# Lain-Iwakuro/Plonky2-Demo

Hardware: AMD Instinct MI355X
Metric: proofs/sec for m=64 matmul circuit (full prove(), PoseidonGoldilocksConfig, standard_recursion_config) (higher is better)
Workload: dtype u64 (Goldilocks, 64-bit modular integer)

## Files before the change

plonky2_demo_amd/csrc/merkle.hip:

```cpp
#include "context.hpp"
#include "poseidon.cuh"
#include "keccak.cuh"
#include "host_circuit.hpp"
#include <cstring>
#include <memory>

struct gl_merkle {
    gl_ctx* ctx = nullptr;
    GlMerkle tree;
    gl_t* leaves = nullptr;
    size_t num_leaves = 0, leaf_len = 0;
};

#define GL_COOP_MAX_NODES_DEFAULT 8192u
#define GL_COOP_MAX_NODES_THROUGHPUT 1024u
static uint32_t gl_coop_max_nodes() {
    static const long env = [] { const char* e = getenv("GL_COOP_MAX_NODES"); return e ? (long)strtoul(e, nullptr, 10) : -1L; }();
    if (env >= 0) return (uint32_t)env;
    return gl_proofs_in_flight.load(std::memory_order_relaxed) > 2 ? GL_COOP_MAX_NODES_THROUGHPUT : GL_COOP_MAX_NODES_DEFAULT;
}

__device__ __forceinline__ uint32_t d_bitrev(uint32_t x, uint32_t bits) { return bits ? (__brev(x) >> (32 - bits)) : 0; }

template <int WPE>
__global__ __launch_bounds__(256, WPE) void k_merkle_leaves(const gl_t* __restrict__ base, const uint64_t* __restrict__ offsets,
                                                       uint32_t leaf_len, uint32_t lg_leaves, gl_t* __restrict__ digests) {
    const uint32_t n = 1u << lg_leaves, gid = blockIdx.x * blockDim.x + threadIdx.x, r = gid < n ? gid : n - 1;
    gl_t s[12];
#pragma unroll
    for (int i = 0; i < 12; i++) s[i] = 0;
    if (leaf_len <= 4) {
        for (uint32_t e = 0; e < leaf_len; e++) s[e] = gl_canon(base[offsets[e] + r]);
    } else {
        for (uint32_t e0 = 0; e0 < leaf_len; e0 += 8) {
            const uint32_t c = leaf_len - e0 < 8 ? leaf_len - e0 : 8;
#pragma unroll
            for (int i = 0; i < 8; i++)
                if ((uint32_t)i < c) s[i] = base[offsets[e0 + i] + r];
            psd_permute_layer<PSD_LAYER_HASH>(s);
        }
    }
    if (gid >= n) return;
    const uint32_t j = d_bitrev(r, lg_leaves);
    ulonglong2* out = reinterpret_cast<ulonglong2*>(digests + 4ull * j);
    out[0] = make_ulonglong2(gl_canon(s[0]), gl_canon(s[1]));
    out[1] = make_ulonglong2(gl_canon(s[2]), gl_canon(s[3]));
}

__global__ __launch_bounds__(256, 5) void k_merkle_level(const gl_t* __restrict__ child, gl_t* __restrict__ parent, uint32_t count) {
    const uint32_t gid = blockIdx.x * blockDim.x + threadIdx.x, i = gid < count ? gid : count - 1;
    const ulonglong2* in = reinterpret_cast<const ulonglong2*>(child + 8ull * i);
    ulonglong2 a = in[0], b = in[1], c = in[2], d = in[3];
    gl_t s[12] = {a.x, a.y, b.x, b.y, c.x, c.y, d.x, d.y, 0, 0, 0, 0};
    psd_permute_layer<PSD_LAYER_HASH>(s);
    if (gid >= count) return;
    ulonglong2* out = reinterpret_cast<ulonglong2*>(parent + 4ull * i);
    out[0] = make_ulonglong2(gl_canon(s[0]), gl_canon(s[1]));
    out[1] = make_ulonglong2(gl_canon(s[2]), gl_canon(s[3]));
}

__global__ __launch_bounds__(256) void k_merkle_level_coop(const gl_t* __restrict__ child, gl_t* __restrict__ parent, uint32_t count) {
    const uint32_t gid = blockIdx.x * blockDim.x + threadIdx.x, node = gid >> 4;
    const int l = (int)(gid & 15);
    if (node >= count) return;
    gl_t s = l < 8 ? child[8ull * node + l] : 0;
    s = psd_coop_permute(s, l);
    if (l < 4) parent[4ull * node + l] = gl_canon(s);
}
__global__ __launch_bounds__(256) void k_merkle_leaves_coop(const gl_t* __restrict__ base, const uint64_t* __restrict__ offsets,
                                                            uint32_t leaf_len, uint32_t lg_leaves, gl_t* __restrict__ digests) {
    const uint32_t gid = blockIdx.x * blockDim.x + threadIdx.x, r = gid >> 4;
    const int l = (int)(gid & 15);
    if (r >= (1u << lg_leaves)) return;
    gl_t s = 0;
    if (leaf_len <= 4) {
        if ((uint32_t)l < leaf_len) s = gl_canon(base[offsets[l] + r]);
    } else {
        for (uint32_t e0 = 0; e0 < leaf_len; e0 += 8) {
            const uint32_t c = leaf_len - e0 < 8 ? leaf_len - e0 : 8;
            if ((uint32_t)l < c) s = base[offsets[e0 + l] + r];
            s = psd_coop_permute(s, l);
        }
    }
    if (l < 4) digests[4ull * d_bitrev(r, lg_leaves) + l] = gl_canon(s);
}

#define GL_TOP_NODES 64u
__global__ __launch_bounds__(1024) void k_merkle_top_coop(gl_t* __restrict__ digests, const uint64_t* __restrict__ lev_off, uint32_t first_level,
                                                          uint32_t num_levels, uint32_t nodes_first ) {
    const uint32_t sub = blockIdx.x, g = threadIdx.x >> 4;
    const int l = (int)(threadIdx.x & 15);
    uint32_t nodes = nodes_first;
    for (uint32_t lev = first_level; lev < num_levels; lev++, nodes >>= 1) {
        const gl_t* child = digests + 4 * lev_off[lev - 1] + 8ull * sub * nodes;
        gl_t* parent = digests + 4 * lev_off[lev] + 4ull * sub * nodes;
        if (g < nodes) {
            gl_t s = l < 8 ? child[8ull * g + l] : 0;
            s = psd_coop_permute(s, l);
            if (l < 4) parent[4ull * g + l] = gl_canon(s);
        }
        __syncthreads();
    }
}

template <int LAYER, bool CANON>
__global__ __launch_bounds__(64, 5) void k_poseidon_states(gl_t* states, size_t count) {
    const size_t gid = (size_t)blockIdx.x * blockDim.x + threadIdx.x, i = gid < count ? gid : count - 1;
    gl_t s[12];
#pragma unroll
    for (int k = 0; k < 12; k++) s[k] = states[12 * i + k];
    psd_permute_layer<LAYER>(s);
// ... 72 lines not shown
        for (uint32_t e = 0; e < len; e++) h[e] = gl_canon(row[e]);
    } else {
        kck_state s;
        kck_absorb_leaf(s, len, [&](uint32_t e) { return row[e]; });
        kck_digest25(s, h);
    }
    for (int i = 0; i < 4; i++) out[4 * r + i] = h[i];
}

static int kck_merkle_levels(gl_ctx* c, const gl_t* base, const uint64_t* d_off, uint32_t leaf_len, uint32_t lg_leaves, uint32_t cap_height, GlMerkle* out) {
    const uint32_t levels = lg_leaves - cap_height + 1, n = 1u << lg_leaves;
    c->timing_begin("merkle_leaf_hash");
    hipLaunchKernelGGL(k_kck_leaves, dim3((n + 255) / 256), dim3(256), 0, c->stream, base, d_off, leaf_len, lg_leaves, out->level_ptr(0));
    c->timing_end();
    GL_CHECK_HIP(hipGetLastError());
    c->timing_begin("merkle_levels");
    uint32_t top_first = levels;
    for (uint32_t l = 1; l < levels; l++)
        if (((1u << (lg_leaves - l)) >> cap_height) <= GL_KCK_TOP_NODES) { top_first = l; break; }
    const uint64_t* d_lev_off = nullptr;
    if (top_first < levels && levels - top_first >= 2) GL_TRY(c->get_offsets_table(out->level_off.data(), out->level_off.size(), &d_lev_off));
    else top_first = levels;
    for (uint32_t l = 1; l < top_first; l++) {
        const uint32_t cnt = 1u << (lg_leaves - l);
        hipLaunchKernelGGL(k_kck_level, dim3((cnt + 255) / 256), dim3(256), 0, c->stream, out->level_ptr(l - 1), out->level_ptr(l), cnt);
    }
    if (top_first < levels)
        hipLaunchKernelGGL(k_kck_top, dim3(1u << cap_height), dim3(64), 0, c->stream, out->digests, d_lev_off, top_first, levels, (1u << (lg_leaves - top_first)) >> cap_height);
    c->timing_end();
    GL_CHECK_HIP(hipGetLastError());
    return GL_OK;
}

int gl_merkle_build(gl_ctx* c, const gl_t* base, const uint64_t* host_offsets, uint32_t leaf_len, uint32_t lg_leaves,
                    uint32_t cap_height, GlMerkle* out, uint32_t hasher) {
    GL_REQUIRE(c && base && host_offsets && out, GL_ERR_ARG, "gl_merkle_build: null argument");
    GL_REQUIRE_HASHER(hasher, "gl_merkle_build");
    GL_REQUIRE(cap_height <= lg_leaves, GL_ERR_ARG, "cap_height should be at most log2(leaves.len())");
    GL_REQUIRE(lg_leaves <= 30 && leaf_len >= 1 && leaf_len <= 4096, GL_ERR_ARG, "gl_merkle_build: unsupported shape");
    GL_TRY(c->activate());
    out->lg_leaves = lg_leaves; out->cap_height = cap_height; out->leaf_len = leaf_len; out->hasher = hasher;
    const uint32_t levels = lg_leaves - cap_height + 1;
    out->level_off.resize(levels);
    uint64_t off = 0;
    for (uint32_t l = 0; l < levels; l++) { out->level_off[l] = off; off += uint64_t(1) << (lg_leaves - l); }
    out->total_digests = off;
    GL_TRY(c->pool_alloc(off * 4 * sizeof(gl_t), (void**)&out->digests));
    const uint64_t* d_off = nullptr;
    GL_TRY(c->get_offsets_table(host_offsets, leaf_len, &d_off));
    if (hasher == GL_HASHER_KECCAK) return kck_merkle_levels(c, base, d_off, leaf_len, lg_leaves, cap_height, out);
    const uint32_t n = 1u << lg_leaves;
    const uint32_t coop = gl_coop_max_nodes();
    c->timing_begin("merkle_leaf_hash");
    if (n <= coop) hipLaunchKernelGGL(k_merkle_leaves_coop, dim3((n * 16 + 255) / 256), dim3(256), 0, c->stream, base, d_off, leaf_len, lg_leaves, out->level_ptr(0));
    else {
        static const int wpe = [] { const char* e = getenv("GL_LEAF_WPE"); return e ? atoi(e) : 5; }();
        auto kern = wpe >= 8 ? k_merkle_leaves<8> : wpe == 7 ? k_merkle_leaves<7> : wpe == 6 ? k_merkle_leaves<6> : wpe == 4 ? k_merkle_leaves<4> : k_merkle_leaves<5>;
        hipLaunchKernelGGL(kern, dim3((n + 255) / 256), dim3(256), 0, c->stream, base, d_off, leaf_len, lg_leaves, out->level_ptr(0));
    }
    c->timing_end();
    GL_CHECK_HIP(hipGetLastError());
    c->timing_begin("merkle_levels");
    uint32_t top_first = levels;
    if (coop > 0)
        for (uint32_t l = 1; l < levels; l++)
            if (((1u << (lg_leaves - l)) >> cap_height) <= GL_TOP_NODES && ((1u << (lg_leaves - l)) >> cap_height) >= 1) { top_first = l; break; }
    const uint64_t* d_lev_off = nullptr;
    if (top_first < levels && levels - top_first >= 2) GL_TRY(c->get_offsets_table(out->level_off.data(), out->level_off.size(), &d_lev_off));
    else top_first = levels;
    for (uint32_t l = 1; l < top_first; l++) {
        const uint32_t cnt = 1u << (lg_leaves - l);
        if (cnt <= coop) hipLaunchKernelGGL(k_merkle_level_coop, dim3((cnt * 16 + 255) / 256), dim3(256), 0, c->stream, out->level_ptr(l - 1), out->level_ptr(l), cnt);
        else hipLaunchKernelGGL(k_merkle_level, dim3((cnt + 255) / 256), dim3(256), 0, c->stream, out->level_ptr(l - 1), out->level_ptr(l), cnt);
    }
    if (top_first < levels)
        hipLaunchKernelGGL(k_merkle_top_coop, dim3(1u << cap_height), dim3(1024), 0, c->stream, out->digests, d_lev_off, top_first, levels,
                           (1u << (lg_leaves - top_first)) >> cap_height);
    c->timing_end();
    GL_CHECK_HIP(hipGetLastError());
    return GL_OK;
}
void gl_merkle_release(gl_ctx* c, GlMerkle* m) {
    if (m && m->digests) { c->pool_release(m->digests); m->digests = nullptr; }
}

extern "C" int gl_poseidon_permute(gl_ctx* c, uint64_t* d_states, size_t count) try {
    GL_REQUIRE(c && d_states, GL_ERR_ARG, "null argument");
    if (!count) return GL_OK;
    GL_TRY(c->activate());
    hipLaunchKernelGGL((k_poseidon_states<PSD_LAYER_HASH, true>), dim3((unsigned)((count + 63) / 64)), dim3(64), 0, c->stream, d_states, count);
    GL_CHECK_HIP(hipGetLastError());
    return GL_OK;
} catch (...) { return gl_caught(); }
extern "C" int gl_poseidon_permute_raw(gl_ctx* c, uint64_t* d_states, size_t count, int layer) try {
    GL_REQUIRE(c && d_states && (layer == PSD_LAYER_VALU || layer == PSD_LAYER_MFMA), GL_ERR_ARG, "bad argument");
    if (!count) return GL_OK;
    GL_TRY(c->activate());
    if (layer == PSD_LAYER_MFMA)
        hipLaunchKernelGGL((k_poseidon_states<PSD_LAYER_MFMA, false>), dim3((unsigned)((count + 63) / 64)), dim3(64), 0, c->stream, d_states, count);
    else
        hipLaunchKernelGGL((k_poseidon_states<PSD_LAYER_VALU, false>), dim3((unsigned)((count + 63) / 64)), dim3(64), 0, c->stream, d_states, count);
    GL_CHECK_HIP(hipGetLastError());
    return GL_OK;
} catch (...) { return gl_caught(); }
extern "C" int gl_hash_rows_h(gl_ctx* c, uint32_t hasher, const uint64_t* d_rows, size_t count, size_t len, uint64_t* d_out) try {
    GL_REQUIRE_HASHER(hasher, "gl_hash_rows_h");
    if (hasher == GL_HASHER_POSEIDON) return gl_hash_rows(c, d_rows, count, len, d_out);
    GL_REQUIRE(c && d_rows && d_out && len >= 1 && len <= 0xFFFFFFFFu, GL_ERR_ARG, "bad argument");
    if (!count) return GL_OK;
    GL_TRY(c->activate());
    hipLaunchKernelGGL(k_kck_hash_rows, dim3((unsigned)((count + 63) / 64)), dim3(64), 0, c->stream, d_rows, count, (uint32_t)len, d_out);
    GL_CHECK_HIP(hipGetLastError());
    return GL_OK;
} catch (...) { return gl_caught(); }
extern "C" int gl_hash_rows(gl_ctx* c, const uint64_t* d_rows, size_t count, size_t len, uint64_t* d_out) try {
    GL_REQUIRE(c && d_rows && d_out && len >= 1, GL_ERR_ARG, "bad argument");
    if (!count) return GL_OK;
    GL_TRY(c->activate());
    hipLaunchKernelGGL(k_hash_rows, dim3((unsigned)((count + 63) / 64)), dim3(64), 0, c->stream, d_rows, count, (uint32_t)len, d_out);
    GL_CHECK_HIP(hipGetLastError());
    return GL_OK;
} catch (...) { return gl_caught(); }

__global__ void k_rows_to_natural_cols(const gl_t* rows, uint32_t lg_rows, uint32_t cols, gl_t* out) {
    const uint64_t idx = (uint64_t)blockIdx.x * blockDim.x + threadIdx.x;
    const uint64_t nrows = uint64_t(1) << lg_rows;
// ... 72 lines not shown
```

plonky2_demo_amd/csrc/prove.hip:

```cpp
#include "context.hpp"
#include "host_circuit.hpp"
#include "fri_instance.hpp"
#include "prover_kernels.cuh"
#include "proof.hpp"
#include <cstring>
#include <memory>

using glhost::HostChallenger;
using glhost::HostCircuit;

static constexpr size_t DS_BYTES = size_t(1) << 20, DS_WORDS = DS_BYTES / sizeof(gl_t);
static constexpr size_t DS_APOW = 0, DS_APOW_WORDS = 2 * GLQ_MAX_TERMS;
static constexpr size_t DS_ZH = DS_APOW + DS_APOW_WORDS, DS_ZH_WORDS = 8;
static constexpr size_t DS_POW = DS_ZH + DS_ZH_WORDS, DS_POW_WORDS = 1;
static constexpr size_t DS_OPEN = 4096, DS_OPEN_MAX = 4096, DS_OPEN_WORDS = 2 * DS_OPEN_MAX;
static_assert(DS_POW + DS_POW_WORDS <= DS_OPEN && DS_OPEN + DS_OPEN_WORDS <= DS_WORDS, "dev_small slices overlap or do not fit");

struct gl_circuit {
    gl_ctx* ctx = nullptr;
    gl_circuit_desc desc;
    size_t n = 0;
    gl_batch* cs_batch = nullptr;
    gl_t* d_sigmas = nullptr;
    gl_t* d_l0_coset = nullptr;
// ... 441 lines not shown
    f.nnext = f.cols.size() - f.nopen;
    return f;
}

struct gl_fri {
    gl_ctx* ctx = nullptr;
    gl_fri_params params;
    std::vector<const gl_batch*> oracles;
    size_t n = 0;
    uint32_t lgN = 0;
    unsigned round = 0;
    bool committed = false;
    std::unique_ptr<DevBuf> cur_vals;
    std::unique_ptr<DevBuf> coef;
    size_t cur_n = 0; uint32_t cur_lgN = 0; gl_t shift = GL_MULT_GENERATOR;
    std::vector<std::unique_ptr<MerkleHolder>> trees;
    std::vector<std::unique_ptr<DevBuf>> vals;
    std::vector<uint32_t> lg;
    std::vector<const gl_t*> h_cols; std::vector<gl_t> h_apow;
    std::vector<const gl_t*> h_listed_cols; std::vector<gl_t> h_listed_apow;
};
extern "C" void gl_fri_free(gl_fri* f) noexcept {
    if (!f) return;
    gl_ctx* ctx = f->ctx;
    if (ctx) (void)gl_stream_wait(ctx->stream);
    delete f;
    gl_ctx_release(ctx);
}
static gl_fri_params fri_params_of(const gl_circuit_desc& d) {
    gl_fri_params p;
    p.degree_bits = d.degree_bits; p.rate_bits = d.rate_bits; p.cap_height = d.cap_height; p.proof_of_work_bits = d.proof_of_work_bits;
    p.num_query_rounds = d.num_query_rounds; p.num_fri_rounds = d.num_fri_rounds;
    for (int r = 0; r < 8; r++) p.fri_arity_bits[r] = d.fri_arity_bits[r];
    p.hiding = d.zero_knowledge; p.hasher = d.hasher;
    return p;
}
static int fri_combine(gl_ctx* ctx, const gl_circuit* cir, const gl_batch* const batches[4], const uint64_t zeta_in[2], const uint64_t alpha_in[2], gl_fri** out) {
    GL_TRY(check_phase_args(ctx, cir));
    GL_REQUIRE(batches && zeta_in && alpha_in && out, GL_ERR_ARG, "gl_fri_combine: null argument");
    const gl_circuit_desc& d = cir->desc;
    const size_t n = cir->n, N = n << d.rate_bits;
    const size_t want[4] = {d.num_constants + 80, 135, 20 + 2 * (size_t)d.num_lookup_polys, 16};
    for (int o = 0; o < 4; o++) GL_TRY(check_batch(cir, batches[o], want[o], "gl_fri_combine: oracle order is constants||sigmas, wires, Z||partial products(||lookups), quotient"));
    FriOpenings op = fri_openings(batches);
    const size_t nopen = op.nopen, nnext = op.nnext;
    hipStream_t st = ctx->stream;
    std::unique_ptr<gl_fri, void (*)(gl_fri*)> f(new gl_fri(), gl_fri_free);
    f->ctx = ctx; ctx->retain(); f->params = fri_params_of(d); f->n = n; f->lgN = d.degree_bits + d.rate_bits;
    f->oracles.assign(batches, batches + 4);
    const gl2_t zeta = gl2_make(gl_canon(zeta_in[0]), gl_canon(zeta_in[1])), fri_alpha = gl2_make(gl_canon(alpha_in[0]), gl_canon(alpha_in[1]));
    const gl2_t gzeta = gl2_canon(gl2_scalar(zeta, gl_host_root_of_unity(d.degree_bits)));
    f->coef.reset(new DevBuf(ctx)); GL_TRY(f->coef->alloc(2 * n * sizeof(gl_t)));
    {
        DevBuf d_F(ctx), d_heads(ctx), d_cols(ctx), d_apow(ctx);
        const uint32_t seg_len = (uint32_t)(n / 1024 > 32 ? n / 1024 : (n >= 32 ? 32 : n));
        const uint32_t nseg = (uint32_t)((n + seg_len - 1) / seg_len);
        GL_TRY(d_F.alloc(2 * n * sizeof(gl_t)));
        GL_TRY(d_heads.alloc(2 * (size_t)nseg * sizeof(gl_t)));
        GL_TRY(d_cols.alloc((nopen + nnext) * sizeof(gl_t*)));
        GL_TRY(d_apow.alloc(2 * (nopen + nnext) * sizeof(gl_t)));
        std::vector<const gl_t*>& cols = f->h_cols;
        cols = std::move(op.cols);
        std::vector<gl_t>& apow = f->h_apow; apow.assign(2 * (nopen + nnext), 0);
        { gl2_t x = gl2_make(1, 0); for (size_t j = 0; j < nopen; j++) { apow[2 * j] = x.a; apow[2 * j + 1] = x.b; x = gl2_canon(gl2_mul(x, fri_alpha)); } }
        gl2_t shift = gl2_make(1, 0);
        { gl2_t x = gl2_make(1, 0); for (size_t j = 0; j < nnext; j++) { apow[2 * (nopen + j)] = x.a; apow[2 * (nopen + j) + 1] = x.b; x = gl2_canon(gl2_mul(x, fri_alpha)); } shift = x; }
        GL_TRY(h2d_async(ctx, d_cols.p, cols.data(), cols.size() * sizeof(gl_t*)));
        GL_TRY(h2d_async(ctx, d_apow.p, apow.data(), apow.size() * sizeof(gl_t)));
        gl_t* Fa = d_F.as<gl_t>(); gl_t* Fb = Fa + n;
        gl_t* Qa = f->coef->as<gl_t>(); gl_t* Qb = Qa + n;
        const unsigned gb = (unsigned)((n + 63) / 64), sb = (nseg + 63) / 64;
        ctx->timing_begin("reduce batch + divide by linear");
        hipLaunchKernelGGL(k_fri_combine, dim3(gb), dim3(256), 0, st, d_cols.as<const gl_t*>(), d_apow.as<gl_t>(), (uint32_t)nopen, (uint32_t)n, Fa, Fb);
        hipLaunchKernelGGL(k_div_linear_heads, dim3(sb), dim3(64), 0, st, Fa, Fb, (uint32_t)n, seg_len, zeta.a, zeta.b, d_heads.as<gl_t>());
        hipLaunchKernelGGL(k_div_linear_carries, dim3(1), dim3(1024), 0, st, d_heads.as<gl_t>(), (uint32_t)n, seg_len, zeta.a, zeta.b);
        hipLaunchKernelGGL(k_div_linear_apply, dim3(sb), dim3(64), 0, st, Fa, Fb, (uint32_t)n, seg_len, zeta.a, zeta.b, d_heads.as<gl_t>(), shift.a, shift.b, Qa, Qb, 0);
        hipLaunchKernelGGL(k_fri_combine, dim3(gb), dim3(256), 0, st, d_cols.as<const gl_t*>() + nopen, d_apow.as<gl_t>() + 2 * nopen, (uint32_t)nnext, (uint32_t)n, Fa, Fb);
        hipLaunchKernelGGL(k_div_linear_heads, dim3(sb), dim3(64), 0, st, Fa, Fb, (uint32_t)n, seg_len, gzeta.a, gzeta.b, d_heads.as<gl_t>());
        hipLaunchKernelGGL(k_div_linear_carries, dim3(1), dim3(1024), 0, st, d_heads.as<gl_t>(), (uint32_t)n, seg_len, gzeta.a, gzeta.b);
        hipLaunchKernelGGL(k_div_linear_apply, dim3(sb), dim3(64), 0, st, Fa, Fb, (uint32_t)n, seg_len, gzeta.a, gzeta.b, d_heads.as<gl_t>(), (gl_t)1, (gl_t)0, Qa, Qb, 1);
        ctx->timing_end();
        GL_CHECK_HIP(hipGetLastError());
    }
    f->cur_vals.reset(new DevBuf(ctx)); GL_TRY(f->cur_vals->alloc(2 * N * sizeof(gl_t)));
    GL_TRY(gl_ntt_run(ctx, f->coef->as<gl_t>(), n, (uint32_t)n, f->cur_vals->as<gl_t>(), N, f->lgN, 2, false, GL_MULT_GENERATOR, 0, 1));
    f->cur_n = n; f->cur_lgN = f->lgN;
    *out = f.release();
    return GL_OK;
}
extern "C" int gl_fri_combine(gl_ctx* ctx, const gl_circuit* cir, const gl_batch* const batches[4], const uint64_t zeta_in[2], const uint64_t alpha_in[2], gl_fri** out) try {
    GL_TRY(check_phase_api(ctx, cir));
    return fri_combine(ctx, cir, batches, zeta_in, alpha_in, out);
} catch (...) { return gl_caught(); }
extern "C" int gl_fri_commit_round(gl_fri* f, uint64_t* h_cap_out) try {
    GL_REQUIRE(f && h_cap_out, GL_ERR_ARG, "gl_fri_commit_round: null argument");
    GL_REQUIRE(f->round < f->params.num_fri_rounds && !f->committed, GL_ERR_ARG, "gl_fri_commit_round: no round left to commit (call gl_fri_fold first)");
    gl_ctx* ctx = f->ctx;
    GL_TRY(ctx->activate());
    const uint32_t ab = f->params.fri_arity_bits[f->round], arity = 1u << ab;
    const size_t curN = size_t(1) << f->cur_lgN;
    std::vector<uint64_t> offs(2 * arity);
    for (uint32_t k = 0; k < arity; k++)
        for (uint32_t cpt = 0; cpt < 2; cpt++) offs[2 * k + cpt] = (uint64_t)cpt * curN + (uint64_t)host_bitrev32(k, ab) * (curN >> ab);
    std::unique_ptr<MerkleHolder> tree(new MerkleHolder(ctx));
    GL_TRY(gl_merkle_build(ctx, f->cur_vals->as<gl_t>(), offs.data(), 2 * arity, f->cur_lgN - ab, f->params.cap_height, &tree->m, f->params.hasher));
    GL_TRY(d2h(ctx, h_cap_out, tree->m.level_ptr(tree->m.num_levels() - 1), (size_t(4) << f->params.cap_height) * sizeof(gl_t)));
    f->trees.push_back(std::move(tree));
    f->committed = true;
    return GL_OK;
} catch (...) { return gl_caught(); }
extern "C" int gl_fri_fold(gl_fri* f, const uint64_t beta_in[2]) try {
    GL_REQUIRE(f && beta_in, GL_ERR_ARG, "gl_fri_fold: null argument");
    GL_REQUIRE(f->committed, GL_ERR_ARG, "gl_fri_fold: commit the round first");
    gl_ctx* ctx = f->ctx;
    GL_TRY(ctx->activate());
    const uint32_t ab = f->params.fri_arity_bits[f->round], arity = 1u << ab;
    const gl2_t beta = gl2_make(gl_canon(beta_in[0]), gl_canon(beta_in[1]));
    const size_t next_n = f->cur_n >> ab;
    GL_REQUIRE(next_n >= 1, GL_ERR_INTERNAL, "FRI fold below one coefficient");
    std::unique_ptr<DevBuf> next(new DevBuf(ctx));
    GL_TRY(next->alloc(2 * next_n * sizeof(gl_t)));
    ctx->timing_begin("fold codewords in the commitment phase");
    hipLaunchKernelGGL(k_fri_fold, dim3((unsigned)((next_n + 255) / 256)), dim3(256), 0, ctx->stream, f->coef->as<gl_t>(), f->coef->as<gl_t>() + f->cur_n,
                       (uint32_t)next_n, arity, beta.a, beta.b, next->as<gl_t>(), next->as<gl_t>() + next_n);
    ctx->timing_end();
    GL_CHECK_HIP(hipGetLastError());
    const gl_t next_shift = gl_canon(gl_exp(f->shift, arity));
    const uint32_t next_lgN = f->cur_lgN - ab;
    std::unique_ptr<DevBuf> next_vals(new DevBuf(ctx));
    GL_TRY(next_vals->alloc(2 * (size_t(1) << next_lgN) * sizeof(gl_t)));
    GL_TRY(gl_ntt_run(ctx, next->as<gl_t>(), next_n, (uint32_t)next_n, next_vals->as<gl_t>(), size_t(1) << next_lgN, next_lgN, 2, false, next_shift, 0, 1));
    f->vals.reserve(f->vals.size() + 1); f->lg.reserve(f->lg.size() + 1);
    f->vals.push_back(std::move(f->cur_vals)); f->lg.push_back(f->cur_lgN);
// ... 25 lines not shown
    GL_REQUIRE(ctx && sponge_state && witness && (input_buffer || !input_len), GL_ERR_ARG, "gl_pow_grind: null argument");
    GL_REQUIRE(input_len < 8 && min_leading_zeros <= 40, GL_ERR_ARG, "gl_pow_grind: the witness must fit the rate (input_len < 8), at most 40 bits of work");
    GL_TRY(ctx->activate());
    hipStream_t st = ctx->stream;
    GL_TRY(ctx->ensure_dev_small(DS_BYTES));
    unsigned long long* d_res = (unsigned long long*)(ctx->dev_small + DS_POW);
    GlPowParams pw;
    for (int i = 0; i < 12; i++) pw.state[i] = hasher == GL_HASHER_KECCAK ? gl_canon(sponge_state[i]) : sponge_state[i];
    for (uint32_t i = 0; i < input_len; i++) pw.state[i] = hasher == GL_HASHER_KECCAK ? gl_canon(input_buffer[i]) : input_buffer[i];
    pw.pos = input_len; pw.min_leading_zeros = min_leading_zeros; pw.result = d_res;
    static const int pow_window_env = [] { const char* e = getenv("GL_POW_WINDOW_LOG"); return e ? atoi(e) : 99; }();
    const int wlog = pow_window_env != 99 ? pow_window_env : (gl_proofs_in_flight.load(std::memory_order_relaxed) > 2 ? 0 : 1);
    const int wbits = (int)min_leading_zeros + wlog < 8 ? 8 : (int)min_leading_zeros + wlog;
    const uint64_t batch = wbits >= 30 ? (uint64_t(1) << 30) : (uint64_t(1) << wbits);
    unsigned long long res = ~0ull;
    ctx->timing_begin("find proof-of-work witness");
    for (uint64_t base = 0; base < GL_P; base += batch) {
        GL_CHECK_HIP(hipMemsetAsync(d_res, 0xFF, sizeof(unsigned long long), st));
        pw.base = base; pw.count = (GL_P - base < batch) ? GL_P - base : batch;
        if (hasher == GL_HASHER_KECCAK) hipLaunchKernelGGL(k_kck_pow_grind, dim3((unsigned)((pw.count + 255) / 256)), dim3(256), 0, st, pw);
        else hipLaunchKernelGGL(k_pow_grind, dim3((unsigned)((pw.count + 255) / 256)), dim3(256), 0, st, pw);
        GL_CHECK_HIP(hipGetLastError());
        GL_TRY(d2h(ctx, &res, d_res, sizeof res));
        if (res != ~0ull) break;
    }
    ctx->timing_end();
    GL_REQUIRE(res != ~0ull, GL_ERR_INTERNAL, "Proof of work failed. This is highly unlikely!");
    *witness = (uint64_t)res;
    return GL_OK;
} catch (...) { return gl_caught(); }

static int fri_query_blob(gl_fri* f, const uint32_t* x_index, uint32_t nq, std::vector<uint8_t>& o) {
    gl_ctx* ctx = f->ctx;
    const gl_fri_params& d = f->params;
    const size_t no = f->oracles.size();
    hipStream_t st = ctx->stream;
    const uint32_t lgN = f->lgN;
    const size_t N = size_t(1) << lgN;
    GL_REQUIRE(f->round == d.num_fri_rounds && !f->committed, GL_ERR_ARG, "gl_fri_query: reduction rounds not finished");
    for (uint32_t q = 0; q < nq; q++) GL_REQUIRE(x_index[q] < N, GL_ERR_ARG, "gl_fri_query: query index out of range");
    struct Piece { size_t off, words; };
    std::vector<Piece> row_piece(no), path_piece(no), fleaf_piece(d.num_fri_rounds), fpath_piece(d.num_fri_rounds);
    size_t total = 0;
    const uint32_t init_levels = lgN - d.cap_height;
    for (size_t o2 = 0; o2 < no; o2++) {
        row_piece[o2] = {total, nq * f->oracles[o2]->leaf_len()}; total += row_piece[o2].words;
        path_piece[o2] = {total, (size_t)nq * init_levels * 4}; total += path_piece[o2].words;
    }
    for (unsigned r = 0; r < d.num_fri_rounds; r++) {
        const uint32_t ab = d.fri_arity_bits[r], lv = f->lg[r] - ab - d.cap_height;
        fleaf_piece[r] = {total, (size_t)nq * (2u << ab)}; total += fleaf_piece[r].words;
        fpath_piece[r] = {total, (size_t)nq * lv * 4}; total += fpath_piece[r].words;
    }
    DevBuf d_stage(ctx), d_idx(ctx);
    GL_TRY(d_stage.alloc((total + 8) * sizeof(gl_t)));
    GL_TRY(d_idx.alloc((size_t)nq * (2 + d.num_fri_rounds) * sizeof(uint32_t)));
    std::vector<uint32_t> idx_host((size_t)nq * (2 + d.num_fri_rounds));
    for (uint32_t q = 0; q < nq; q++) { idx_host[q] = x_index[q]; idx_host[nq + q] = host_bitrev32(x_index[q], lgN); }
    {
        std::vector<uint32_t> xi(x_index, x_index + nq);
        for (unsigned r = 0; r < d.num_fri_rounds; r++) for (uint32_t q = 0; q < nq; q++) { xi[q] >>= d.fri_arity_bits[r]; idx_host[(size_t)(2 + r) * nq + q] = xi[q]; }
    }
    GL_TRY(h2d_async(ctx, d_idx.p, idx_host.data(), idx_host.size() * sizeof(uint32_t)));
    const uint32_t* d_leaf = d_idx.as<uint32_t>();
    const uint32_t* d_rows = d_leaf + nq;
    gl_t* stage = d_stage.as<gl_t>();
    ctx->timing_begin("FRI query gathers");
    for (size_t o2 = 0; o2 < no; o2++) {
        const gl_batch* b = f->oracles[o2];
        const uint64_t* d_lo = nullptr;
        GL_TRY(ctx->get_offsets_table(b->tree.level_off.data(), b->tree.level_off.size(), &d_lo));
        unsigned cnt = nq * (unsigned)b->leaf_len();
        hipLaunchKernelGGL(k_gather_rows, dim3((cnt + 255) / 256), dim3(256), 0, st, b->lde, (uint64_t)N, (uint32_t)b->leaf_len(), d_rows, nq, stage + row_piece[o2].off);
        cnt = nq * init_levels * 4;
        if (cnt) hipLaunchKernelGGL(k_gather_paths, dim3((cnt + 255) / 256), dim3(256), 0, st, b->tree.digests, d_lo, init_levels, d_leaf, nq, stage + path_piece[o2].off);
    }
    for (unsigned r = 0; r < d.num_fri_rounds; r++) {
        const uint32_t ab = d.fri_arity_bits[r], lv = f->lg[r] - ab - d.cap_height;
        const GlMerkle& t = f->trees[r]->m;
        const uint64_t* d_lo = nullptr;
        GL_TRY(ctx->get_offsets_table(t.level_off.data(), t.level_off.size(), &d_lo));
        const gl_t* va = f->vals[r]->as<gl_t>(); const gl_t* vb = va + (size_t(1) << f->lg[r]);
        const uint32_t* d_fl = d_idx.as<uint32_t>() + (size_t)(2 + r) * nq;
        unsigned cnt = nq << ab;
        hipLaunchKernelGGL(k_gather_fri_leaves, dim3((cnt + 255) / 256), dim3(256), 0, st, va, vb, f->lg[r], ab, d_fl, nq, stage + fleaf_piece[r].off);
        cnt = nq * lv * 4;
        if (cnt) hipLaunchKernelGGL(k_gather_paths, dim3((cnt + 255) / 256), dim3(256), 0, st, t.digests, d_lo, lv, d_fl, nq, stage + fpath_piece[r].off);
    }
    ctx->timing_end();
    GL_CHECK_HIP(hipGetLastError());
    std::vector<gl_t> host_stage(total + 8);
    GL_TRY(d2h(ctx, host_stage.data(), stage, total * sizeof(gl_t)));
    for (uint32_t q = 0; q < nq; q++) {
        for (size_t oi = 0; oi < no; oi++) {
            const size_t nc = f->oracles[oi]->leaf_len();
            put_words(o, host_stage.data() + row_piece[oi].off + (size_t)q * nc, nc);
            o.push_back((uint8_t)init_levels);
            put_hashes(o, d.hasher, host_stage.data() + path_piece[oi].off + (size_t)q * init_levels * 4, init_levels);
        }
        for (unsigned r = 0; r < d.num_fri_rounds; r++) {
            const uint32_t ab = d.fri_arity_bits[r], lv = f->lg[r] - ab - d.cap_height;
            put_words(o, host_stage.data() + fleaf_piece[r].off + (size_t)q * (2u << ab), 2u << ab);
            o.push_back((uint8_t)lv);
            put_hashes(o, d.hasher, host_stage.data() + fpath_piece[r].off + (size_t)q * lv * 4, lv);
        }
    }
    return GL_OK;
}
extern "C" int gl_fri_query(gl_fri* f, const uint32_t* x_index, uint32_t num_queries, uint8_t* h_blob, size_t cap_bytes, size_t* num_bytes) try {
    GL_REQUIRE(f && x_index && num_bytes, GL_ERR_ARG, "gl_fri_query: null argument");
    GL_REQUIRE(num_queries >= 1 && num_queries <= 256, GL_ERR_ARG, "gl_fri_query: 1..256 queries");
    GL_TRY(f->ctx->activate());
    std::vector<uint8_t> blob;
    GL_TRY(fri_query_blob(f, x_index, num_queries, blob));
    *num_bytes = blob.size();
    if (!h_blob) return GL_OK;
    GL_REQUIRE(cap_bytes >= blob.size(), GL_ERR_ARG, "gl_fri_query: output too small");
    memcpy(h_blob, blob.data(), blob.size());
    return GL_OK;
} catch (...) { return gl_caught(); }

static_assert(GLF_MAX_POINTS == GL_MAX_FRI_BATCHES, "the kernels' point table holds one entry per batch");
static int check_instance_batches(gl_ctx* ctx, const gl_fri_params& p, const gl_fri_instance& in, const gl_batch* const* batches) {
    GL_REQUIRE(batches, GL_ERR_ARG, "FRI openings: null batch list");
    for (uint32_t o = 0; o < in.num_oracles; o++) {
        const gl_batch* b = batches[o];
        GL_REQUIRE(b && b->ctx && b->ctx->device == ctx->device, GL_ERR_ARG, "FRI openings: a null batch, or one on another device");
        GL_REQUIRE(b->n == (size_t(1) << p.degree_bits) && b->rate_bits == p.rate_bits && b->cap_height == p.cap_height && b->ncols == in.oracle_num_polys[o],
                   GL_ERR_ARG, "FRI openings: a batch whose degree, rate_bits, cap_height or column count differs from params / instance");
        GL_REQUIRE(b->hasher == p.hasher, GL_ERR_ARG, "a batch committed under another hasher than the params'");
        GL_REQUIRE(b->salt == glfri::salt_of(p, in, o), GL_ERR_ARG, "FRI openings: a batch is salted where the instance is not blinded (or the reverse)");
    }
    return GL_OK;
}
static int fri_combine_instance(gl_ctx* ctx, const gl_fri_params* params, const gl_fri_instance* instance, const gl_batch* const* batches, const uint64_t alpha_in[2], gl_fri** out,
                                bool per_batch = false) {
    GL_REQUIRE(ctx && alpha_in && out, GL_ERR_ARG, "gl_fri_combine_instance: null argument");
    GL_TRY(glfri::check(params, instance, true));
    const gl_fri_params& p = *params; const gl_fri_instance& in = *instance;
    GL_TRY(check_instance_batches(ctx, p, in, batches));
    GL_TRY(ctx->activate());
// ... 362 lines not shown
```

plonky2_demo_amd/csrc/prover_kernels.cuh:

```cuda
#pragma once
#include "gl64.cuh"
#include "poseidon.cuh"
#include "keccak.cuh"
#include "gates.hpp"
#include "../../include/plonky2_mi355x.h"

#define GLP_MAX_ROUTED 80
#define GLP_CHUNKS 10

struct GlPermParams {
    const gl_t* wires;
    const gl_t* sigmas;
    const gl_t* xpow_lo; const gl_t* xpow_hi;
    gl_t k_is[GLP_MAX_ROUTED];
    gl_t betas[2], gammas[2];
    uint32_t n;
    uint32_t k_is_powers_of_7;
    gl_t* chunk_prod;
    gl_t* row_prod;
};

__device__ __forceinline__ gl_t glp_pow2level(const gl_t* lo, const gl_t* hi, uint32_t e) {
    return gl_mul(lo[e & 2047], hi[e >> 11]);
}
// ... 850 lines not shown
    const uint32_t lo = s * seg, hi = (lo + seg < n) ? lo + seg : n;
    gl2_t b[B];
#pragma unroll
    for (int t = 0; t < B; t++) b[t] = gl2_make(carries[2 * ((size_t)t * nseg + s)], carries[2 * ((size_t)t * nseg + s) + 1]);
    for (uint32_t k = hi; k > lo; k--) {
        gl2_t q = gl2_make(0, 0);
#pragma unroll
        for (int t = 0; t < B; t++) {
            q = gl2_add(q, gl2_mul(b[t], gl2_make(pt.scale[t][0], pt.scale[t][1])));
            b[t] = gl2_add(gl2_mul(b[t], gl2_make(pt.z[t][0], pt.z[t][1])), gl2_make(F[(size_t)(2 * t) * n + k - 1], F[(size_t)(2 * t + 1) * n + k - 1]));
        }
        qa[k - 1] = gl_canon(q.a); qb[k - 1] = gl_canon(q.b);
    }
}

__global__ __launch_bounds__(256) void k_fri_fold(const gl_t* ia, const gl_t* ib, uint32_t n_out, uint32_t arity, gl_t ba, gl_t bb, gl_t* oa, gl_t* ob) {
    const uint32_t k = blockIdx.x * blockDim.x + threadIdx.x;
    if (k >= n_out) return;
    const gl2_t beta = gl2_make(ba, bb);
    gl2_t acc = gl2_make(0, 0);
    for (uint32_t i = arity; i-- > 0;) acc = gl2_add(gl2_mul(acc, beta), gl2_make(ia[(size_t)arity * k + i], ib[(size_t)arity * k + i]));
    oa[k] = gl_canon(acc.a); ob[k] = gl_canon(acc.b);
}

struct GlPowParams { gl_t state[12]; uint32_t pos, min_leading_zeros; uint64_t base, count; unsigned long long* result; };
__global__ __launch_bounds__(256, 5) void k_pow_grind(GlPowParams p) {
    const uint64_t idx = (uint64_t)blockIdx.x * blockDim.x + threadIdx.x;
    const uint64_t cand = p.base + idx;
    gl_t s[12];
#pragma unroll
    for (int i = 0; i < 12; i++) s[i] = p.state[i];
#pragma unroll
    for (int i = 0; i < 8; i++) if ((uint32_t)i == p.pos) s[i] = cand;
    psd_permute_layer<PSD_LAYER_HASH>(s);
    const gl_t r = gl_canon(s[7]);
    const uint32_t lz = r ? (uint32_t)__clzll((long long)r) : 64u;
    if (idx < p.count && lz >= p.min_leading_zeros) atomicMin(p.result, (unsigned long long)cand);
}
__global__ __launch_bounds__(256) void k_kck_pow_grind(GlPowParams p) {
    const uint64_t idx = (uint64_t)blockIdx.x * blockDim.x + threadIdx.x;
    if (idx >= p.count) return;
    const uint64_t cand = p.base + idx;
    gl_t s[12], e[8];
#pragma unroll
    for (int i = 0; i < 12; i++) s[i] = p.state[i];
#pragma unroll
    for (int i = 0; i < 8; i++) if ((uint32_t)i == p.pos) s[i] = cand;
    kck_onion<8>(s, e);
    const gl_t r = e[7];
    const uint32_t lz = r ? (uint32_t)__clzll((long long)r) : 64u;
    if (lz >= p.min_leading_zeros) atomicMin(p.result, (unsigned long long)cand);
}

__global__ void k_gather_rows(const gl_t* base, uint64_t stride, uint32_t ncols, const uint32_t* rows, uint32_t nq, gl_t* out) {
    const uint32_t idx = blockIdx.x * blockDim.x + threadIdx.x;
    if (idx >= nq * ncols) return;
    const uint32_t q = idx / ncols, c = idx % ncols;
    out[idx] = base[(uint64_t)c * stride + rows[q]];
}
__global__ void k_gather_paths(const gl_t* digests, const uint64_t* level_off, uint32_t nlevels, const uint32_t* leaves, uint32_t nq, gl_t* out) {
    const uint32_t idx = blockIdx.x * blockDim.x + threadIdx.x;
    if (idx >= nq * nlevels * 4) return;
    const uint32_t k = idx & 3, l = (idx >> 2) % nlevels, q = (idx >> 2) / nlevels;
    out[idx] = digests[4 * (level_off[l] + ((leaves[q] >> l) ^ 1u)) + k];
}
__global__ void k_gather_fri_leaves(const gl_t* va, const gl_t* vb, uint32_t lg_len, uint32_t arity_bits, const uint32_t* leaves, uint32_t nq, gl_t* out) {
    const uint32_t idx = blockIdx.x * blockDim.x + threadIdx.x;
    const uint32_t arity = 1u << arity_bits;
    if (idx >= nq * arity) return;
    const uint32_t q = idx >> arity_bits, k = idx & (arity - 1);
    const uint32_t pos = (leaves[q] << arity_bits) | k;
    const uint32_t nat = lg_len ? (__brev(pos) >> (32 - lg_len)) : 0;
    out[2 * idx] = va[nat]; out[2 * idx + 1] = vb[nat];
}
```

Before: 303.8.

## Fuse Merkle leaf hashing with lower levels and batch multiple levels per kernel

Result: no change. 302.1 (-0.5%).

```diff
diff --git a/plonky2_demo_amd/csrc/merkle.hip b/plonky2_demo_amd/csrc/merkle.hip
--- a/plonky2_demo_amd/csrc/merkle.hip
+++ b/plonky2_demo_amd/csrc/merkle.hip
@@ -57,6 +57,116 @@
     ulonglong2* out = reinterpret_cast<ulonglong2*>(parent + 4ull * i);
     out[0] = make_ulonglong2(gl_canon(s[0]), gl_canon(s[1]));
     out[1] = make_ulonglong2(gl_canon(s[2]), gl_canon(s[3]));
+}
+
+__device__ __forceinline__ uint32_t d_wave_in_group() { return __builtin_amdgcn_readfirstlane(threadIdx.x >> 6); }
+__device__ __forceinline__ uint32_t d_lane_here() {
+    uint32_t l = __builtin_amdgcn_mbcnt_hi(~0u, __builtin_amdgcn_mbcnt_lo(~0u, 0u));
+    asm volatile("" : "+v"(l));
+    return l;
+}
+__device__ __forceinline__ void d_store_digest(gl_t* __restrict__ level, uint32_t i, const gl_t (&d)[4]) {
+    ulonglong2* out = reinterpret_cast<ulonglong2*>(level + 4ull * i);
+    out[0] = make_ulonglong2(d[0], d[1]);
+    out[1] = make_ulonglong2(d[2], d[3]);
+}
+
+template <int WPE>
+__global__ __launch_bounds__(256, WPE) void k_merkle_leaves_fused(const gl_t* __restrict__ base, const uint64_t* __restrict__ offsets,
+                                                                  uint32_t leaf_len, uint32_t lg_leaves, gl_t* __restrict__ digests) {
+    __shared__ gl_t x[16 * 64];
+    const uint32_t n = 1u << lg_leaves, w = d_wave_in_group(), row0 = 64 * blockIdx.x + ((w & 1) << (lg_leaves - 1)) + ((w >> 1) << (lg_leaves - 2));
+    const uint32_t sponge_steps = leaf_len <= 4 ? 0 : (leaf_len + 7) / 8;
+    gl_t s[12];
+#pragma unroll
+    for (int i = 0; i < 12; i++) s[i] = 0;
+    if (leaf_len <= 4)
+#pragma unroll
+        for (int e = 0; e < 4; e++)
+            if ((uint32_t)e < leaf_len) s[e] = gl_canon(base[offsets[e] + row0 + d_lane_here()]);
+    gl_t* level = digests;
+    for (uint32_t step = 0;; step++) {
+        const uint32_t lane = d_lane_here();
+        gl_t in[8] = {0, 0, 0, 0, 0, 0, 0, 0};
+        uint32_t c = 8;
+        bool hash = true;
+        const bool level_input = step >= sponge_steps;
+        if (!level_input) {
+            const uint32_t e0 = 8 * step, r = row0 + lane;
+            c = leaf_len - e0 < 8 ? leaf_len - e0 : 8;
+#pragma unroll
+            for (int i = 0; i < 8; i++)
+                if ((uint32_t)i < c) in[i] = base[offsets[e0 + i] + r];
+        } else {
+            const uint32_t t = step - sponge_steps;
+            const bool mine = w < (4u >> t);
+            const uint32_t B = d_bitrev(64 * blockIdx.x + lane, lg_leaves - 2);
+            gl_t d[4];
+#pragma unroll
+            for (int k = 0; k < 4; k++) d[k] = gl_canon(s[k]);
+            if (mine) d_store_digest(level, (B << (2 - t)) + w, d);
+            if (t == 2) break;
+            if (mine)
+#pragma unroll
+                for (int k = 0; k < 4; k++) x[(4 * (w << t) + k) * 64 + lane] = d[k];
+            __syncthreads();
+            level += 4ull * (n >> t);
+            hash = w < (2u >> t);
+            if (hash)
+#pragma unroll
+                for (int k = 0; k < 8; k++) in[k] = x[(4 * ((2 * w + (k >> 2)) << t) + (k & 3)) * 64 + lane];
+        }
+#pragma unroll
+        for (int i = 0; i < 8; i++)
+            if ((uint32_t)i < c) s[i] = in[i];
+#pragma unroll
+        for (int i = 8; i < 12; i++)
+            if (level_input) s[i] = 0;
+        if (hash) psd_permute_layer<PSD_LAYER_HASH>(s);
+    }
+}
+
+template <int D>
+__global__ __launch_bounds__(256, 5) void k_merkle_levels(const gl_t* __restrict__ child, gl_t* __restrict__ parent, uint32_t count) {
+    static_assert(D == 2 || D == 3, "a level is hashed on whole waves only");
+    __shared__ gl_t x[16 * 64];
+    const uint32_t w = d_wave_in_group();
+    gl_t s[12];
+    {
+        const ulonglong2* in = reinterpret_cast<const ulonglong2*>(child + 8ull * (256 * blockIdx.x + threadIdx.x));
+        const ulonglong2 a = in[0], b = in[1], c = in[2], d = in[3];
+        s[0] = a.x; s[1] = a.y; s[2] = b.x; s[3] = b.y; s[4] = c.x; s[5] = c.y; s[6] = d.x; s[7] = d.y;
+    }
+#pragma unroll
+    for (int k = 8; k < 12; k++) s[k] = 0;
+    gl_t* level = parent;
+    for (uint32_t t = 0;; t++) {
+        if (w >= (4u >> t)) {
+            if (t == D - 1) break;
+            __syncthreads();
+            continue;
+        }
+        psd_permute_layer<PSD_LAYER_HASH>(s);
+        const uint32_t lane = d_lane_here();
+        gl_t d[4];
+#pragma unroll
+        for (int k = 0; k < 4; k++) d[k] = gl_canon(s[k]);
+        d_store_digest(level, (256u >> t) * blockIdx.x + 64 * w + lane, d);
+        if (t == D - 1) break;
+#pragma unroll
+        for (int k = 0; k < 4; k++) x[(4 * (w << t) + k) * 64 + lane] = d[k];
+        __syncthreads();
+        level += 4ull * (count >> t);
+        if (w >= (2u >> t)) continue;
+#pragma unroll
+        for (int e = 0; e < 2; e++) {
+            const uint32_t y = 2 * lane + e, slot = (2 * w + (y >> 6)) << t;
+#pragma unroll
+            for (int k = 0; k < 4; k++) s[4 * e + k] = x[(4 * slot + k) * 64 + (y & 63)];
+        }
+#pragma unroll
+        for (int k = 8; k < 12; k++) s[k] = 0;
+    }
 }
 
 __global__ __launch_bounds__(256) void k_merkle_level_coop(const gl_t* __restrict__ child, gl_t* __restrict__ parent, uint32_t count) {
@@ -235,26 +345,36 @@
     const uint32_t n = 1u << lg_leaves;
     const uint32_t coop = gl_coop_max_nodes();
     c->timing_begin("merkle_leaf_hash");
+    static const int wpe = [] { const char* e = getenv("GL_LEAF_WPE"); return e ? atoi(e) : 5; }();
+    static const int fuse = [] { const char* e = getenv("GL_MERKLE_FUSE"); return e ? atoi(e) : 2; }();
+    const bool fused_leaves = (fuse & 1) && n > coop && n >= 256 && levels >= 3 && wpe == 5;
     if (n <= coop) hipLaunchKernelGGL(k_merkle_leaves_coop, dim3((n * 16 + 255) / 256), dim3(256), 0, c->stream, base, d_off, leaf_len, lg_leaves, out->level_ptr(0));
+    else if (fused_leaves) hipLaunchKernelGGL(k_merkle_leaves_fused<5>, dim3(n / 256), dim3(256), 0, c->stream, base, d_off, leaf_len, lg_leaves, out->digests);
     else {
-        static const int wpe = [] { const char* e = getenv("GL_LEAF_WPE"); return e ? atoi(e) : 5; }();
         auto kern = wpe >= 8 ? k_merkle_leaves<8> : wpe == 7 ? k_merkle_leaves<7> : wpe == 6 ? k_merkle_leaves<6> : wpe == 4 ? k_merkle_leaves<4> : k_merkle_leaves<5>;
         hipLaunchKernelGGL(kern, dim3((n + 255) / 256), dim3(256), 0, c->stream, base, d_off, leaf_len, lg_leaves, out->level_ptr(0));
     }
     c->timing_end();
     GL_CHECK_HIP(hipGetLastError());
     c->timing_begin("merkle_levels");
+    const uint32_t first = fused_leaves ? 3 : 1;
     uint32_t top_first = levels;
     if (coop > 0)
-        for (uint32_t l = 1; l < levels; l++)
+        for (uint32_t l = first; l < levels; l++)
             if (((1u << (lg_leaves - l)) >> cap_height) <= GL_TOP_NODES && ((1u << (lg_leaves - l)) >> cap_height) >= 1) { top_first = l; break; }
     const uint64_t* d_lev_off = nullptr;
     if (top_first < levels && levels - top_first >= 2) GL_TRY(c->get_offsets_table(out->level_off.data(), out->level_off.size(), &d_lev_off));
     else top_first = levels;
-    for (uint32_t l = 1; l < top_first; l++) {
+    for (uint32_t l = first; l < top_first;) {
         const uint32_t cnt = 1u << (lg_leaves - l);
-        if (cnt <= coop) hipLaunchKernelGGL(k_merkle_level_coop, dim3((cnt * 16 + 255) / 256), dim3(256), 0, c->stream, out->level_ptr(l - 1), out->level_ptr(l), cnt);
+        uint32_t run = 0;
+        while (l + run < top_first && (cnt >> run) > coop) run++;
+        const uint32_t depth = !(fuse & 2) || cnt < 256 || run < 2 ? 1 : run == 2 || run == 4 ? 2 : 3;
+        if (depth == 3) hipLaunchKernelGGL(k_merkle_levels<3>, dim3(cnt / 256), dim3(256), 0, c->stream, out->level_ptr(l - 1), out->level_ptr(l), cnt);
+        else if (depth == 2) hipLaunchKernelGGL(k_merkle_levels<2>, dim3(cnt / 256), dim3(256), 0, c->stream, out->level_ptr(l - 1), out->level_ptr(l), cnt);
+        else if (cnt <= coop) hipLaunchKernelGGL(k_merkle_level_coop, dim3((cnt * 16 + 255) / 256), dim3(256), 0, c->stream, out->level_ptr(l - 1), out->level_ptr(l), cnt);
         else hipLaunchKernelGGL(k_merkle_level, dim3((cnt + 255) / 256), dim3(256), 0, c->stream, out->level_ptr(l - 1), out->level_ptr(l), cnt);
+        l += depth;
     }
     if (top_first < levels)
         hipLaunchKernelGGL(k_merkle_top_coop, dim3(1u << cap_height), dim3(1024), 0, c->stream, out->digests, d_lev_off, top_first, levels,
```

## Fuse FRI two-point combine/divide and batch query gathers into single launches

Applied to the files above, without the earlier changes.

After: 311.9 before, 315.6 after (median of 6 runs). 1.01x the previous value.

```diff
diff --git a/plonky2_demo_amd/csrc/prove.hip b/plonky2_demo_amd/csrc/prove.hip
--- a/plonky2_demo_amd/csrc/prove.hip
+++ b/plonky2_demo_amd/csrc/prove.hip
@@ -517,33 +517,41 @@
     const gl2_t gzeta = gl2_canon(gl2_scalar(zeta, gl_host_root_of_unity(d.degree_bits)));
     f->coef.reset(new DevBuf(ctx)); GL_TRY(f->coef->alloc(2 * n * sizeof(gl_t)));
     {
-        DevBuf d_F(ctx), d_heads(ctx), d_cols(ctx), d_apow(ctx);
+        DevBuf d_F(ctx), d_heads(ctx), d_cols(ctx), d_wts(ctx);
         const uint32_t seg_len = (uint32_t)(n / 1024 > 32 ? n / 1024 : (n >= 32 ? 32 : n));
         const uint32_t nseg = (uint32_t)((n + seg_len - 1) / seg_len);
-        GL_TRY(d_F.alloc(2 * n * sizeof(gl_t)));
-        GL_TRY(d_heads.alloc(2 * (size_t)nseg * sizeof(gl_t)));
-        GL_TRY(d_cols.alloc((nopen + nnext) * sizeof(gl_t*)));
-        GL_TRY(d_apow.alloc(2 * (nopen + nnext) * sizeof(gl_t)));
+        GL_TRY(d_F.alloc(4 * n * sizeof(gl_t)));
+        GL_TRY(d_heads.alloc(4 * (size_t)nseg * sizeof(gl_t)));
+        GL_TRY(d_cols.alloc(nopen * sizeof(gl_t*)));
+        GL_TRY(d_wts.alloc(4 * nopen * sizeof(gl_t)));
         std::vector<const gl_t*>& cols = f->h_cols;
         cols = std::move(op.cols);
-        std::vector<gl_t>& apow = f->h_apow; apow.assign(2 * (nopen + nnext), 0);
-        { gl2_t x = gl2_make(1, 0); for (size_t j = 0; j < nopen; j++) { apow[2 * j] = x.a; apow[2 * j + 1] = x.b; x = gl2_canon(gl2_mul(x, fri_alpha)); } }
+        std::vector<gl_t>& wts = f->h_apow; wts.assign(4 * nopen, 0);
+        { gl2_t x = gl2_make(1, 0); for (size_t j = 0; j < nopen; j++) { wts[4 * j] = x.a; wts[4 * j + 1] = x.b; x = gl2_canon(gl2_mul(x, fri_alpha)); } }
         gl2_t shift = gl2_make(1, 0);
-        { gl2_t x = gl2_make(1, 0); for (size_t j = 0; j < nnext; j++) { apow[2 * (nopen + j)] = x.a; apow[2 * (nopen + j) + 1] = x.b; x = gl2_canon(gl2_mul(x, fri_alpha)); } shift = x; }
-        GL_TRY(h2d_async(ctx, d_cols.p, cols.data(), cols.size() * sizeof(gl_t*)));
-        GL_TRY(h2d_async(ctx, d_apow.p, apow.data(), apow.size() * sizeof(gl_t)));
-        gl_t* Fa = d_F.as<gl_t>(); gl_t* Fb = Fa + n;
+        {
+            gl2_t x = gl2_make(1, 0);
+            for (size_t k = 0; k < nnext; k++) {
+                const size_t j = k < 2 ? op.zs() + k : op.lookups() + (k - 2);
+                GL_REQUIRE(cols[j] == cols[nopen + k], GL_ERR_INTERNAL, "gl_fri_combine: a polynomial opened at g zeta is not where it is opened at zeta");
+                wts[4 * j + 2] = x.a; wts[4 * j + 3] = x.b;
+                x = gl2_canon(gl2_mul(x, fri_alpha));
+            }
+            shift = x;
+        }
+        GlFriPoints pt = {};
+        pt.z[0][0] = zeta.a; pt.z[0][1] = zeta.b; pt.scale[0][0] = shift.a; pt.scale[0][1] = shift.b;
+        pt.z[1][0] = gzeta.a; pt.z[1][1] = gzeta.b; pt.scale[1][0] = 1;
+        GL_TRY(h2d_async(ctx, d_cols.p, cols.data(), nopen * sizeof(gl_t*)));
+        GL_TRY(h2d_async(ctx, d_wts.p, wts.data(), wts.size() * sizeof(gl_t)));
+        gl_t* F = d_F.as<gl_t>();
         gl_t* Qa = f->coef->as<gl_t>(); gl_t* Qb = Qa + n;
         const unsigned gb = (unsigned)((n + 63) / 64), sb = (nseg + 63) / 64;
         ctx->timing_begin("reduce batch + divide by linear");
-        hipLaunchKernelGGL(k_fri_combine, dim3(gb), dim3(256), 0, st, d_cols.as<const gl_t*>(), d_apow.as<gl_t>(), (uint32_t)nopen, (uint32_t)n, Fa, Fb);
-        hipLaunchKernelGGL(k_div_linear_heads, dim3(sb), dim3(64), 0, st, Fa, Fb, (uint32_t)n, seg_len, zeta.a, zeta.b, d_heads.as<gl_t>());
-        hipLaunchKernelGGL(k_div_linear_carries, dim3(1), dim3(1024), 0, st, d_heads.as<gl_t>(), (uint32_t)n, seg_len, zeta.a, zeta.b);
-        hipLaunchKernelGGL(k_div_linear_apply, dim3(sb), dim3(64), 0, st, Fa, Fb, (uint32_t)n, seg_len, zeta.a, zeta.b, d_heads.as<gl_t>(), shift.a, shift.b, Qa, Qb, 0);
-        hipLaunchKernelGGL(k_fri_combine, dim3(gb), dim3(256), 0, st, d_cols.as<const gl_t*>() + nopen, d_apow.as<gl_t>() + 2 * nopen, (uint32_t)nnext, (uint32_t)n, Fa, Fb);
-        hipLaunchKernelGGL(k_div_linear_heads, dim3(sb), dim3(64), 0, st, Fa, Fb, (uint32_t)n, seg_len, gzeta.a, gzeta.b, d_heads.as<gl_t>());
-        hipLaunchKernelGGL(k_div_linear_carries, dim3(1), dim3(1024), 0, st, d_heads.as<gl_t>(), (uint32_t)n, seg_len, gzeta.a, gzeta.b);
-        hipLaunchKernelGGL(k_div_linear_apply, dim3(sb), dim3(64), 0, st, Fa, Fb, (uint32_t)n, seg_len, gzeta.a, gzeta.b, d_heads.as<gl_t>(), (gl_t)1, (gl_t)0, Qa, Qb, 1);
+        hipLaunchKernelGGL(k_fri_combine_points<2>, dim3(gb), dim3(256), 0, st, d_cols.as<const gl_t*>(), d_wts.as<gl_t>(), (uint32_t)nopen, (uint32_t)n, F);
+        hipLaunchKernelGGL(k_div_points_heads, dim3(sb, 2), dim3(64), 0, st, F, (uint32_t)n, seg_len, pt, d_heads.as<gl_t>());
+        hipLaunchKernelGGL(k_div_points_carries, dim3(1, 2), dim3(1024), 0, st, d_heads.as<gl_t>(), (uint32_t)n, seg_len, pt);
+        hipLaunchKernelGGL(k_div_points_apply<2>, dim3(sb), dim3(64), 0, st, F, (uint32_t)n, seg_len, pt, d_heads.as<gl_t>(), Qa, Qb);
         ctx->timing_end();
         GL_CHECK_HIP(hipGetLastError());
     }
@@ -675,28 +683,30 @@
         fleaf_piece[r] = {total, (size_t)nq * (2u << ab)}; total += fleaf_piece[r].words;
         fpath_piece[r] = {total, (size_t)nq * lv * 4}; total += fpath_piece[r].words;
     }
-    DevBuf d_stage(ctx), d_idx(ctx);
-    GL_TRY(d_stage.alloc((total + 8) * sizeof(gl_t)));
-    GL_TRY(d_idx.alloc((size_t)nq * (2 + d.num_fri_rounds) * sizeof(uint32_t)));
-    std::vector<uint32_t> idx_host((size_t)nq * (2 + d.num_fri_rounds));
+    const size_t max_pieces = 2 * (no + d.num_fri_rounds), idx_words = (size_t)nq * (2 + d.num_fri_rounds);
+    GL_REQUIRE(max_pieces <= GLG_MAX_PIECES, GL_ERR_INTERNAL, "gl_fri_query: more pieces than the gather table holds");
+    static_assert(sizeof(GlGatherPiece) == 64, "the table is laid out in 64-byte entries ahead of the indices");
+    std::vector<uint64_t> up_host(max_pieces * (sizeof(GlGatherPiece) / 8) + (idx_words + 1) / 2);
+    GlGatherPiece* pieces = reinterpret_cast<GlGatherPiece*>(up_host.data());
+    uint32_t* idx_host = reinterpret_cast<uint32_t*>(pieces + max_pieces);
     for (uint32_t q = 0; q < nq; q++) { idx_host[q] = x_index[q]; idx_host[nq + q] = host_bitrev32(x_index[q], lgN); }
     {
         std::vector<uint32_t> xi(x_index, x_index + nq);
         for (unsigned r = 0; r < d.num_fri_rounds; r++) for (uint32_t q = 0; q < nq; q++) { xi[q] >>= d.fri_arity_bits[r]; idx_host[(size_t)(2 + r) * nq + q] = xi[q]; }
     }
-    GL_TRY(h2d_async(ctx, d_idx.p, idx_host.data(), idx_host.size() * sizeof(uint32_t)));
-    const uint32_t* d_leaf = d_idx.as<uint32_t>();
-    const uint32_t* d_rows = d_leaf + nq;
-    gl_t* stage = d_stage.as<gl_t>();
-    ctx->timing_begin("FRI query gathers");
+    uint32_t npieces = 0, nblocks = 0;
+    auto add_piece = [&](uint32_t kind, const gl_t* src, const gl_t* src2, const uint64_t* level_off, uint64_t stride, uint32_t a, uint32_t b2, size_t count,
+                         size_t idx_off, size_t out_off) {
+        if (!count) return;
+        pieces[npieces++] = GlGatherPiece{src, src2, level_off, stride, (uint64_t)out_off, kind, a, b2, (uint32_t)count, (uint32_t)idx_off, 0};
+        nblocks += (uint32_t)((count + 255) / 256);
+    };
     for (size_t o2 = 0; o2 < no; o2++) {
         const gl_batch* b = f->oracles[o2];
         const uint64_t* d_lo = nullptr;
         GL_TRY(ctx->get_offsets_table(b->tree.level_off.data(), b->tree.level_off.size(), &d_lo));
-        unsigned cnt = nq * (unsigned)b->leaf_len();
-        hipLaunchKernelGGL(k_gather_rows, dim3((cnt + 255) / 256), dim3(256), 0, st, b->lde, (uint64_t)N, (uint32_t)b->leaf_len(), d_rows, nq, stage + row_piece[o2].off);
-        cnt = nq * init_levels * 4;
-        if (cnt) hipLaunchKernelGGL(k_gather_paths, dim3((cnt + 255) / 256), dim3(256), 0, st, b->tree.digests, d_lo, init_levels, d_leaf, nq, stage + path_piece[o2].off);
+        add_piece(GLG_ROWS, b->lde, nullptr, nullptr, (uint64_t)N, (uint32_t)b->leaf_len(), 0, (size_t)nq * b->leaf_len(), nq, row_piece[o2].off);
+        add_piece(GLG_PATHS, b->tree.digests, nullptr, d_lo, 0, init_levels, 0, (size_t)nq * init_levels * 4, 0, path_piece[o2].off);
     }
     for (unsigned r = 0; r < d.num_fri_rounds; r++) {
         const uint32_t ab = d.fri_arity_bits[r], lv = f->lg[r] - ab - d.cap_height;
@@ -704,12 +714,18 @@
         const uint64_t* d_lo = nullptr;
         GL_TRY(ctx->get_offsets_table(t.level_off.data(), t.level_off.size(), &d_lo));
         const gl_t* va = f->vals[r]->as<gl_t>(); const gl_t* vb = va + (size_t(1) << f->lg[r]);
-        const uint32_t* d_fl = d_idx.as<uint32_t>() + (size_t)(2 + r) * nq;
-        unsigned cnt = nq << ab;
-        hipLaunchKernelGGL(k_gather_fri_leaves, dim3((cnt + 255) / 256), dim3(256), 0, st, va, vb, f->lg[r], ab, d_fl, nq, stage + fleaf_piece[r].off);
-        cnt = nq * lv * 4;
-        if (cnt) hipLaunchKernelGGL(k_gather_paths, dim3((cnt + 255) / 256), dim3(256), 0, st, t.digests, d_lo, lv, d_fl, nq, stage + fpath_piece[r].off);
-    }
+        add_piece(GLG_FRI_LEAVES, va, vb, nullptr, 0, ab, f->lg[r], (size_t)nq << ab, (size_t)(2 + r) * nq, fleaf_piece[r].off);
+        add_piece(GLG_PATHS, t.digests, nullptr, d_lo, 0, lv, 0, (size_t)nq * lv * 4, (size_t)(2 + r) * nq, fpath_piece[r].off);
+    }
+    DevBuf d_stage(ctx), d_up(ctx);
+    GL_TRY(d_stage.alloc((total + 8) * sizeof(gl_t)));
+    GL_TRY(d_up.alloc(up_host.size() * sizeof(uint64_t)));
+    GL_TRY(h2d_async(ctx, d_up.p, up_host.data(), up_host.size() * sizeof(uint64_t)));
+    gl_t* stage = d_stage.as<gl_t>();
+    ctx->timing_begin("FRI query gathers");
+    if (nblocks)
+        hipLaunchKernelGGL(k_gather_pieces, dim3(nblocks), dim3(256), 0, st, d_up.as<GlGatherPiece>(), npieces,
+                           reinterpret_cast<const uint32_t*>(d_up.as<GlGatherPiece>() + max_pieces), stage);
     ctx->timing_end();
     GL_CHECK_HIP(hipGetLastError());
     std::vector<gl_t> host_stage(total + 8);
diff --git a/plonky2_demo_amd/csrc/prover_kernels.cuh b/plonky2_demo_amd/csrc/prover_kernels.cuh
--- a/plonky2_demo_amd/csrc/prover_kernels.cuh
+++ b/plonky2_demo_amd/csrc/prover_kernels.cuh
@@ -926,24 +926,38 @@
     if (lz >= p.min_leading_zeros) atomicMin(p.result, (unsigned long long)cand);
 }
 
-__global__ void k_gather_rows(const gl_t* base, uint64_t stride, uint32_t ncols, const uint32_t* rows, uint32_t nq, gl_t* out) {
-    const uint32_t idx = blockIdx.x * blockDim.x + threadIdx.x;
-    if (idx >= nq * ncols) return;
-    const uint32_t q = idx / ncols, c = idx % ncols;
-    out[idx] = base[(uint64_t)c * stride + rows[q]];
-}
-__global__ void k_gather_paths(const gl_t* digests, const uint64_t* level_off, uint32_t nlevels, const uint32_t* leaves, uint32_t nq, gl_t* out) {
-    const uint32_t idx = blockIdx.x * blockDim.x + threadIdx.x;
-    if (idx >= nq * nlevels * 4) return;
-    const uint32_t k = idx & 3, l = (idx >> 2) % nlevels, q = (idx >> 2) / nlevels;
-    out[idx] = digests[4 * (level_off[l] + ((leaves[q] >> l) ^ 1u)) + k];
-}
-__global__ void k_gather_fri_leaves(const gl_t* va, const gl_t* vb, uint32_t lg_len, uint32_t arity_bits, const uint32_t* leaves, uint32_t nq, gl_t* out) {
-    const uint32_t idx = blockIdx.x * blockDim.x + threadIdx.x;
-    const uint32_t arity = 1u << arity_bits;
-    if (idx >= nq * arity) return;
-    const uint32_t q = idx >> arity_bits, k = idx & (arity - 1);
-    const uint32_t pos = (leaves[q] << arity_bits) | k;
-    const uint32_t nat = lg_len ? (__brev(pos) >> (32 - lg_len)) : 0;
-    out[2 * idx] = va[nat]; out[2 * idx + 1] = vb[nat];
-}
+enum { GLG_ROWS = 0, GLG_PATHS = 1, GLG_FRI_LEAVES = 2 };
+#define GLG_MAX_PIECES 32
+struct GlGatherPiece {
+    const gl_t* src; const gl_t* src2;
+    const uint64_t* level_off;
+    uint64_t stride, out_off;
+    uint32_t kind, a, b, count, idx_off, pad_;
+};
+__global__ __launch_bounds__(256) void k_gather_pieces(const GlGatherPiece* __restrict__ pieces, uint32_t npieces, const uint32_t* __restrict__ idx,
+                                                       gl_t* __restrict__ out) {
+    uint32_t blk = blockIdx.x, p = 0;
+    for (; p < npieces; p++) {
+        const uint32_t nb = (pieces[p].count + 255) / 256;
+        if (blk < nb) break;
+        blk -= nb;
+    }
+    if (p == npieces) return;
+    const GlGatherPiece& pc = pieces[p];
+    const uint32_t i = blk * 256 + threadIdx.x;
+    if (i >= pc.count) return;
+    const uint32_t* ix = idx + pc.idx_off;
+    gl_t* o = out + pc.out_off;
+    if (pc.kind == GLG_ROWS) {
+        const uint32_t q = i / pc.a, c = i % pc.a;
+        o[i] = pc.src[(uint64_t)c * pc.stride + ix[q]];
+    } else if (pc.kind == GLG_PATHS) {
+        const uint32_t k = i & 3, l = (i >> 2) % pc.a, q = (i >> 2) / pc.a;
+        o[i] = pc.src[4 * (pc.level_off[l] + ((ix[q] >> l) ^ 1u)) + k];
+    } else {
+        const uint32_t q = i >> pc.a, k = i & ((1u << pc.a) - 1);
+        const uint32_t pos = (ix[q] << pc.a) | k;
+        const uint32_t nat = pc.b ? (__brev(pos) >> (32 - pc.b)) : 0;
+        o[2 * i] = pc.src[nat]; o[2 * i + 1] = pc.src2[nat];
+    }
+}
```
